# foxeng/libzseek

Measured on AMD Instinct MI355X. Metric: decompressed GB/s whole-node + achieved %HBM-read, LZ4 64KiB frames, higher is better.
Workload: dtype u8; 1 GPU; config2: LZ4 64KiB frames, 4 GiB synthetic per GPU, full-range decode, compressed image resident in HBM; frame_bytes=65536, frames_per_gpu=65536, decoded_bytes_total=4294967296, decoded_bytes_per_gpu=4294967296, compressed_bytes_per_gpu=2124820559, parallelism=one GPU

## Files before the change

### libzseek_amd/csrc/lz4_lean.hip

```cpp
#include <hip/hip_runtime.h>
#include <stdint.h>
#include <stdio.h>

#include "lz4_dev.h"
#include "zsk_internal.h"

namespace zsk {

namespace {

using namespace lz4d;

constexpr uint32_t kItemExt = 0x80000000u;
constexpr uint32_t kItemPos = 0x3FFFFFFFu;
constexpr uint32_t kLW = 4;
constexpr uint32_t kRing = 256;
constexpr uint32_t kMirror = 256, kSink = 272, kIBuf = 304;
constexpr uint32_t kStride = 560;
constexpr uint32_t kFlush = 8;
constexpr uint32_t kOff = 0x80000000u;

enum : uint32_t { P_TOKEN = 0, P_LEXT, P_OFF, P_MEXT, P_BHDR, P_END, P_DONE };

struct Fill {
    u32x4 a, b, c, d;
    uint32_t x;
    bool h2;
};

struct Lane {
    __amdgpu_buffer_rsrc_t cin, irs;
    uint32_t cx0;
    uint32_t clen, dlen;
    uint32_t ring;
    uint32_t fill, avail;
    uint32_t ph;
    int32_t st;
    uint32_t ip, op, fail_op;
    uint32_t csz_flag;
    uint64_t csize;
    uint32_t indep, bsid, max_block;
    uint32_t iend, oend, floor_, bop;
    uint32_t mlim;
    uint32_t tok, lsrc, nlit;
    uint32_t acc, moff;
    uint32_t stop;
    uint32_t ib, k, cap;
    uint32_t kf;
    uint32_t ia, ibw, ia2, ib2, nk;
    uint32_t cnt[22];
    uint32_t why;
};

constexpr int kLeanStats = 22;
__device__ unsigned long long g_lean_stats[kLeanStats];

__device__ __forceinline__ uint32_t lds_u32(uint32_t a)
{
    return *reinterpret_cast<const __attribute__((address_space(3))) uint32_t *>(
        (__attribute__((address_space(3))) void *)(uintptr_t)a);
}

__device__ __forceinline__ uint32_t lds_u8(uint32_t a)
{
    return *reinterpret_cast<const __attribute__((address_space(3))) uint8_t *>(
        (__attribute__((address_space(3))) void *)(uintptr_t)a);
}

template <typename T>
__device__ __forceinline__ __attribute__((address_space(3))) T *lp(uint32_t a)
{
    return (__attribute__((address_space(3))) T *)(uintptr_t)a;
}

__device__ __forceinline__ void lds_w128(uint32_t a, u32x4 v)
{
    *reinterpret_cast<__attribute__((address_space(3))) u32x4 *>(
        (__attribute__((address_space(3))) void *)(uintptr_t)a) = v;
}

__device__ __forceinline__ uint32_t raddr(const Lane &L, uint32_t x)
{
    return L.ring + (x & (kRing - 1));
}

__device__ __forceinline__ bool have(const Lane &L, uint32_t p, uint32_t n)
{
    return L.cx0 + p + n <= L.avail;
}

__device__ __forceinline__ uint32_t rb(const Lane &L, uint32_t p)
{
    return lds_u8(raddr(L, L.cx0 + p));
}

__device__ __forceinline__ uint32_t r4(const Lane &L, uint32_t p)
{
    const uint32_t x = L.cx0 + p;
    const uint32_t a = L.ring + (x & (kRing - 4));
    return __builtin_amdgcn_alignbyte(lds_u32(a + 4), lds_u32(a), x & 3);
}

__device__ __forceinline__ void ring_put(const Lane &L, uint32_t x, u32x4 a, u32x4 b, bool on)
{
    const uint32_t i = x & (kRing - 1);
    lds_w128(L.ring + (on ? i : kSink), a);
    lds_w128(L.ring + (on ? i + 16 : kSink + 16), b);
    lds_w128(L.ring + ((on && i == 0) ? kMirror : kSink), a);
}

__device__ __forceinline__ uint32_t rd32(const Lane &L, uint32_t p)
{
    return rb(L, p) | (rb(L, p + 1) << 8) | (rb(L, p + 2) << 16) | (rb(L, p + 3) << 24);
}

__device__ __forceinline__ u32x4 bload16(__amdgpu_buffer_rsrc_t r, uint32_t x)
{
    return __builtin_bit_cast(u32x4, __builtin_amdgcn_raw_buffer_load_b128(r, x, 0, 0));
}

__device__ __forceinline__ void finish(Lane &L, int32_t st)
{
    L.st = st;
    L.ph = P_DONE;
}

__device__ __forceinline__ void fail_block(Lane &L)
{
    const bool direct = (L.dlen - L.bop) >= L.max_block;
    const int32_t bits = (int32_t)((L.bsid - 4) << ST_BSID_SHIFT);
    finish(L, (direct ? (ST_GENERIC | ST_DIRECT_FLAG) : ST_DECOMPRESS_FAILED) | ST_BLOCK_FAIL_FLAG | bits);
}

__device__ __forceinline__ bool emit(Lane &L, uint32_t lsrc, uint32_t lit, uint32_t off, uint32_t ml)
{
    if (L.k + 2 > L.cap)
        return false;
    if (lit > 255 || ml > 258) {
        L.ia = lsrc | kItemExt;
        L.ibw = off;
        L.ia2 = lit;
        L.ib2 = ml;
        L.nk = 2;
    } else {
        L.ia = lsrc;
        L.ibw = off | (lit << 16) | ((ml ? ml - 3 : 0) << 24);
        L.ia2 = 0;
        L.ib2 = 0;
        L.nk = 1;
    }
    return true;
}

__device__ __forceinline__ int32_t hdr_status(Lane &L)
{
    const uint32_t clen = L.clen;
    if (clen < 7)
        return ST_HDR_INCOMPLETE;
    const uint32_t magic = rd32(L, 0);
    if ((magic & 0xFFFFFFF0u) == 0x184D2A50u)
        return ST_SHORT_FRAME;
    if (magic != kLz4Magic)
        return ST_FRAME_TYPE;
    const uint32_t flg = rb(L, 4), bd = rb(L, 5);
    if (flg & 0x14)
        return ST_NOT_RUN;
    const uint32_t dictid = flg & 1;
    if ((flg >> 1) & 1)
        return ST_RESERVED;
    if (((flg >> 6) & 3) != 1)
        return ST_VERSION;
    const uint32_t csz = (flg >> 3) & 1;
    const uint32_t hdr = 7 + (csz ? 8 : 0) + (dictid ? 4 : 0);
    if (clen < hdr)
        return ST_HDR_INCOMPLETE;
    const uint32_t bsid = (bd >> 4) & 7;
    if ((bd >> 7) & 1)
        return ST_RESERVED;
    if (bsid < 4)
        return ST_MAXBLOCK;
    if (bd & 15)
        return ST_RESERVED;
    const uint32_t n = hdr - 5;
    uint32_t acc = 0x165667B1u + n;
    uint32_t i = 0;
    for (; i + 4 <= n; i += 4) {
        acc += rd32(L, 4 + i) * 0xC2B2AE3Du;
        acc = ((acc << 17) | (acc >> 15)) * 0x27D4EB2Fu;
    }
    for (; i < n; i++) {
        acc += rb(L, 4 + i) * 0x165667B1u;
        acc = ((acc << 11) | (acc >> 21)) * 0x9E3779B1u;
    }
    acc ^= acc >> 15;
    acc *= 0x85EBCA77u;
    acc ^= acc >> 13;
    acc *= 0xC2B2AE3Du;
    acc ^= acc >> 16;
    if (((acc >> 8) & 0xFF) != rb(L, hdr - 1))
        return ST_HDR_CHECKSUM;
    L.indep = (flg >> 5) & 1;
    L.csz_flag = csz;
    L.bsid = bsid;
    if (csz)
        L.csize = (uint64_t)rd32(L, 6) | ((uint64_t)rd32(L, 10) << 32);
    L.max_block = 1u << (8 + 2 * bsid);
    L.ip = hdr;
    return -1;
}

template <bool FV = true>
__device__ __forceinline__ bool fast(Lane &L, uint32_t fe, uint32_t pc, u32x4 &fv)
{
    const uint32_t ip = L.ip, ph = L.ph;
    const bool po = ph == P_OFF;
    const uint32_t w = r4(L, ip);
    const uint32_t tok = w & 0xFF, e = (w >> 8) & 0xFF;
    const bool lext = (tok >> 4) == 15;
    const uint32_t lit = lext ? 15 + e : tok >> 4;
    const uint32_t p = ip + (lext ? 2 : 1);
    const uint32_t q = p + lit;
    if (FV)
        fv = *lp<u32x4>(fe + 16 * pc);
    const uint32_t o4q = r4(L, q);
    const uint32_t qq = po ? ip : q;
    const uint32_t o4 = po ? w : o4q;
    const uint32_t mtok = po ? L.tok : tok;
    const uint32_t off = o4 & 0xFFFF, e2 = (o4 >> 16) & 0xFF;
    const bool mext = (mtok & 15) == 15;
    const uint32_t ml = (mext ? 15 + e2 : mtok & 15) + kMinMatch;
    const uint32_t nip = qq + (mext ? 3 : 2);
    const uint32_t lt = po ? L.nlit : lit, ls = po ? L.lsrc : p;
    const uint32_t cop = po ? L.op : L.op + lit;
    const int32_t s_av = (int32_t)(L.avail - (L.cx0 + qq + 3));
    const int32_t s_in = (int32_t)(L.iend - qq - 8);
    const int32_t s_lx = (!po & lext & (e == 255)) ? -1 : 0, s_mx = (int32_t)(273 - ml);
    const int32_t s_mf = po ? 0 : (int32_t)(L.oend - kMfLimit - cop);
    const int32_t s_dl = po ? 0 : (int32_t)(L.dlen - cop);
    const int32_t s_off = min((int32_t)(off - 1), (int32_t)(cop - L.floor_ - off));
    const int32_t s_end = (int32_t)(L.mlim - cop - ml);
    const int32_t s_cap = (int32_t)(min(L.cap, L.kf + 32) - L.k - 2);
    const int32_t s_ph = ((ph == P_TOKEN) | po) ? 0 : -1;
    const int32_t s_t = min(min(s_in, s_dl), min(s_lx, s_mf));
    const int32_t slack = min(min(min(s_av, s_t), min(s_mx, s_off)), min(s_end, min(s_cap, s_ph)));
    const bool go = slack >= 0;
    const bool tok_av = (int32_t)(L.avail - (L.cx0 + ip + 2)) >= 0;
    const bool half = (ph == P_TOKEN) & tok_av & (s_t >= 0) & (s_av < 0);
    L.why = (s_av < 0) | (s_in < 0) << 1 | (s_lx < 0) << 2 | (s_mf < 0) << 3 | (s_mx < 0) << 4 |
            (s_off < 0) << 5 | (s_end < 0) << 6 | (s_cap < 0) << 7 | (!po & (ph != P_TOKEN)) << 8;
    const bool big = (lt > 255) | (ml > 258);
    L.ia = big ? ls | kItemExt : ls;
    L.ibw = big ? off : off | (lt << 16) | ((ml - 3) << 24);
    L.ia2 = lt;
    L.ib2 = ml;
    L.nk = go ? (big ? 2 : 1) : 0;
    L.ip = go ? nip : (half ? q : ip);
    L.op = go ? cop + ml : (half ? cop : L.op);
    L.lsrc = half ? p : L.lsrc;
    L.nlit = half ? lit : L.nlit;
    L.tok = half ? tok : L.tok;
    L.ph = go ? (uint32_t)P_TOKEN : (half ? (uint32_t)P_OFF : ph);
    const bool full = L.k + 2 > L.kf + 32;
    const bool wait = (!tok_av & (ip + 2 <= L.clen)) | full;
    const bool x_wait = (ph != P_END) & ((int32_t)(L.avail - (L.cx0 + ip + 4)) < 0) & (ip + 4 <= L.clen);
    return !go & !half & (ph != P_DONE) & (((ph != P_TOKEN) | po) ? !x_wait & !(po & full) : !wait);
}

__device__ __forceinline__ void lit_done(Lane &L, uint32_t p, uint32_t lit)
{
    if (L.op + lit > L.oend - kMfLimit || L.iend - p < lit + 2 + 1 + kLastLiterals) {
        if (L.iend - p != lit || L.op + lit > L.oend) {
            fail_block(L);
            return;
        }
        if (L.op + lit > L.dlen) {
            finish(L, ST_DST_OVERFLOW);
            return;
        }
        if (!emit(L, p, lit, 0, 0)) {
            finish(L, ST_NOT_RUN);
            return;
        }
        L.op += lit;
        L.ip = L.iend;
        L.ph = P_BHDR;
        return;
    }
    if (L.op + lit > L.dlen) {
        finish(L, ST_DST_OVERFLOW);
        return;
    }
    L.lsrc = p;
    L.nlit = lit;
    L.op += lit;
    L.ip = p + lit;
    L.ph = P_OFF;
}

__device__ __forceinline__ void match_done(Lane &L, uint32_t p, uint32_t off, uint32_t ml)
{
    ml += kMinMatch;
    if (off > L.op - L.floor_) {
        fail_block(L);
        return;
    }
    if (off == 0) {
        finish(L, ST_NOT_RUN);
        return;
    }
    if (L.op + ml > L.oend - kLastLiterals) {
        fail_block(L);
        return;
    }
    if (L.op + ml > L.dlen) {
        finish(L, ST_DST_OVERFLOW);
        return;
    }
    if (!emit(L, L.lsrc, L.nlit, off, ml)) {
        finish(L, ST_NOT_RUN);
        return;
    }
    L.op += ml;
    L.ip = p;
    L.ph = P_TOKEN;
}

__device__ __forceinline__ void slow(Lane &L)
{
    if (L.k + 2 > L.kf + 32)
        return;
    if (L.ph == P_TOKEN) {
        uint32_t p = L.ip;
        if (p >= L.iend) {
            fail_block(L);
            return;
        }
        if (!have(L, p, 1))
            return;
        const uint32_t tok = rb(L, p++);
        L.tok = tok;
        if ((tok >> 4) != 15) {
            lit_done(L, p, tok >> 4);
            return;
        }
        if (L.iend - p <= 15) {
            fail_block(L);
            return;
        }
        L.acc = 15;
        L.ip = p;
        L.ph = P_LEXT;
    }
    if (L.ph == P_LEXT) {
        uint32_t p = L.ip, lit = L.acc, e;
        do {
            if (p >= L.iend) {
                fail_block(L);
                return;
            }
            if (!have(L, p, 1)) {
                L.ip = p;
                L.acc = lit;
                return;
            }
            e = rb(L, p++);
            lit += e;
        } while (e == 255);
        lit_done(L, p, lit);
        return;
    }
    if (L.ph == P_OFF) {
        uint32_t p = L.ip;
        if (!have(L, p, 2))
            return;
        const uint32_t off = rb(L, p) | (rb(L, p + 1) << 8);
        p += 2;
        if ((L.tok & 15) != 15) {
            match_done(L, p, off, L.tok & 15);
            return;
        }
        L.moff = off;
        L.acc = 15;
        L.ip = p;
        L.ph = P_MEXT;
    }
    if (L.ph == P_MEXT) {
        uint32_t p = L.ip, ml = L.acc, e;
        do {
            if (p >= L.iend) {
                fail_block(L);
                return;
            }
            if (!have(L, p, 1)) {
                L.ip = p;
                L.acc = ml;
                return;
            }
            e = rb(L, p++);
            ml += e;
            if (p >= L.iend - (kLastLiterals - 1)) {
                fail_block(L);
                return;
            }
        } while (e == 255);
        match_done(L, p, L.moff, ml);
        return;
    }
    if (L.ph == P_BHDR) {
        if (L.ip == L.stop) {
            finish(L, ST_OK);
            return;
        }
        L.fail_op = L.op;
        if (L.clen - L.ip < 4) {
            finish(L, ST_TRUNCATED);
            return;
        }
        if (!have(L, L.ip, 4))
            return;
        const uint32_t bh = rd32(L, L.ip);
        L.ip += 4;
        if (bh == 0) {
            L.ph = P_END;
        } else {
            const uint32_t bsize = bh & 0x7FFFFFFFu;
            if (bsize > L.max_block) {
                finish(L, ST_MAXBLOCK);
                return;
            }
            if (L.clen - L.ip < bsize) {
                finish(L, ST_TRUNCATED);
                return;
            }
            L.bop = L.op;
            if (bh & 0x80000000u) {
                if (L.op + bsize > L.dlen) {
                    finish(L, ST_DST_OVERFLOW);
                    return;
                }
                if (!emit(L, L.ip, bsize, 0, 0)) {
                    finish(L, ST_NOT_RUN);
                    return;
                }
                L.op += bsize;
                L.ip += bsize;
                return;
            }
            if (bsize == 0) {
                fail_block(L);
                return;
            }
            L.iend = L.ip + bsize;
            L.oend = L.op + L.max_block;
            L.floor_ = L.indep ? L.op : 0;
            L.mlim = min(L.oend - kLastLiterals, L.dlen);
            L.ph = P_TOKEN;
            return;
        }
    }
    if (L.ph == P_END) {
        L.fail_op = L.op;
        if (L.csz_flag && L.csize != L.op)
            finish(L, ST_FRAME_SIZE);
        else
            finish(L, L.op != L.dlen ? ST_SHORT_FRAME : ST_OK);
    }
}

__device__ __forceinline__ uint32_t flush_hand(Lane &L, uint32_t tab)
{
    const bool ready = L.k - L.kf >= 16;
    const uint64_t rm = __ballot(ready);
    const uint32_t j = __builtin_amdgcn_mbcnt_hi((uint32_t)(rm >> 32), __builtin_amdgcn_mbcnt_lo((uint32_t)rm, 0u));
    const bool mine = ready && j < kFlush;
    const uint32_t line = L.ring + kIBuf + 128 * ((L.kf >> 4) & 1);
    *lp<uint64_t>(mine ? tab + 8 * j : tab + 8 * kFlush) = ((uint64_t)(8 * (L.ib + L.kf)) << 32) | line;
    L.kf = mine ? L.kf + 16 : L.kf;
    return min((uint32_t)__builtin_popcountll(rm), kFlush);
}

__device__ __forceinline__ void put_items(Lane &L)
{
    const uint32_t ibuf = L.ring + kIBuf;
    const uint32_t a0 = L.nk ? ibuf + 8 * (L.k & 31) : L.ring + kSink;
    const uint32_t a1 = L.nk == 2 ? ibuf + 8 * ((L.k + 1) & 31) : L.ring + kSink + 8;
    *lp<uint64_t>(a0) = ((uint64_t)L.ibw << 32) | L.ia;
    *lp<uint64_t>(a1) = ((uint64_t)L.ib2 << 32) | L.ia2;
    L.k += L.nk;
    L.nk = 0;
}

__device__ __forceinline__ void fill_retire(Lane &L, const Fill &S)
{
    const bool in = S.x == L.avail;
    ring_put(L, S.x, S.a, S.b, in);
    ring_put(L, S.x + 32, S.c, S.d, in && S.h2);
    L.avail = in ? L.avail + (S.h2 ? 64 : 32) : L.avail;
}

__device__ __forceinline__ void fill_issue(Lane &L, Fill &S, uint32_t need_x, bool live)
{
    const bool jump = need_x >= L.fill;
    L.fill = jump ? need_x & ~31u : L.fill;
    L.avail = jump ? L.fill : L.avail;
    const uint32_t lim = need_x + kRing - 16;
    const bool fl = live & (L.fill < L.cx0 + L.clen) & (L.fill + 32 <= lim);
    const bool f2 = fl & (L.fill + 32 < L.cx0 + L.clen) & (L.fill + 64 <= lim);
    const uint32_t fx = fl ? L.fill : kOff;
    S.x = fx;
    S.h2 = f2;
    S.a = bload16(L.cin, fx);
    S.b = bload16(L.cin, fl ? fx + 16 : kOff);
    S.c = bload16(L.cin, f2 ? fx + 32 : kOff);
    S.d = bload16(L.cin, f2 ? fx + 48 : kOff);
    L.fill = fl ? L.fill + (f2 ? 64 : 32) : L.fill;
}

template <int DIAG>
__device__ __forceinline__ void flush_store(const Lane &L, uint64_t fe, const u32x4 &fv, uint32_t g,
                                            uint32_t pc, uint32_t fcnt)
{
    const uint32_t at = (DIAG & 2) ? 16 * pc : (uint32_t)(fe >> 32) + 16 * pc;
    __builtin_amdgcn_raw_buffer_store_b128(__builtin_bit_cast(u32x4, fv), L.irs,
                                           g < fcnt && !(DIAG & 1) ? at : kOff, 0, 0);
}

template <bool SLOW, bool FILL, int DIAG>
__device__ __forceinline__ void sub(Lane &L, Fill &S, uint32_t lane, uint32_t tab, uint32_t &fcnt)
{
    if (FILL)
        fill_retire(L, S);
    const uint32_t g = lane >> 3, pc = lane & 7;
    const uint64_t fe = *lp<uint64_t>(tab + 8 * (g < fcnt ? g : kFlush));
    u32x4 fv;
    const bool need = fast(L, (uint32_t)fe, pc, fv);
    if (DIAG & 4) {
        L.cnt[0] += L.nk != 0;
        L.cnt[1] += need;
        L.cnt[2] += L.nk == 0 && !need && L.ph != P_DONE;
        L.cnt[3] += L.ph == P_DONE;
        if (need) {
            for (int b = 0; b < 9; b++)
                L.cnt[6 + b] += (L.why >> b) & 1;
            L.cnt[15 + min(L.ph, 6u)] += 1;
        }
    }
    flush_store<DIAG>(L, fe, fv, g, pc, fcnt);
    if (SLOW && __builtin_expect(__ballot(need) != 0, 0)) {
        if (DIAG & 4)
            L.cnt[4] += 1;
        if (need)
            slow(L);
    }
    put_items(L);
    if (!(DIAG & 32)) {
        u32x4 dv;
        (void)fast(L, L.ring + kSink, 0, dv);
        put_items(L);
    }
    wave_lds_sync();
    fcnt = flush_hand(L, tab);
    wave_lds_sync();
    if (!FILL)
        return;
    fill_issue(L, S, L.cx0 + L.ip, L.ph < P_END);
}

__device__ __forceinline__ bool lane_setup(Lane &L, const FrameDesc &d, bool act, uint64_t rb0, uint32_t cap,
                                           const uint8_t *comp, uint64_t *items, uint64_t capacity,
                                           uint64_t clo, uint64_t chi, uint64_t ilo, uint64_t ihi)
{
    const uintptr_t cbase = reinterpret_cast<uintptr_t>(comp + clo) & ~(uintptr_t)31;
    const uint64_t cspan = reinterpret_cast<uintptr_t>(comp + chi) - cbase;
    const uint64_t ispan = (ihi - ilo) * 8;
    const bool fits = cspan < 0x7FFFFF00ull && ispan < 0x7FFFFF00ull;
    L.cin = __builtin_amdgcn_make_buffer_rsrc((void *)cbase, 0, fits ? (int)(uint32_t)((cspan + 3) & ~3ull) : 0,
                                              kRsrcDw3);
    L.irs = __builtin_amdgcn_make_buffer_rsrc((void *)(items + ilo), 0, fits ? (int)(uint32_t)ispan : 0, kRsrcDw3);
    L.ib = (uint32_t)(rb0 - ilo);
    L.cx0 = (uint32_t)(reinterpret_cast<uintptr_t>(comp + d.c_off) - cbase);
    L.clen = d.c_size;
    L.dlen = d.d_size;
    L.fill = L.cx0 & ~31u;
    L.avail = L.fill;
    L.ph = P_BHDR;
    L.st = ST_NOT_RUN;
    L.ip = L.op = L.fail_op = 0;
    L.csz_flag = 0;
    L.csize = 0;
    L.indep = L.bsid = L.max_block = 0;
    L.iend = L.oend = L.floor_ = L.bop = L.mlim = 0;
    L.tok = L.lsrc = L.nlit = L.acc = L.moff = 0;
    L.k = L.kf = 0;
    L.stop = 0xFFFFFFFFu;
    L.cap = cap;
    L.ia = L.ibw = L.ia2 = L.ib2 = L.nk = 0;
    for (int i = 0; i < kLeanStats; i++)
        L.cnt[i] = 0;
    L.why = 0;
    return act && fits && d.c_size <= kItemPos && rb0 + cap <= capacity;
}

__device__ __forceinline__ void head_fill(Lane &L)
{
#pragma unroll
    for (int i = 0; i < 4; i++) {
        const uint32_t fx = L.fill;
        const u32x4 a = bload16(L.cin, fx), b = bload16(L.cin, fx + 16);
        ring_put(L, fx, a, b, true);
        L.fill += 32;
    }
    L.avail = L.fill;
}

template <int DIAG, int D, bool BLK>
__global__ __launch_bounds__(64 * kLW) __attribute__((amdgpu_waves_per_eu(1, 1))) void lz4_lean_kernel(
    const FrameDesc *__restrict__ desc, uint32_t n, const uint8_t *__restrict__ comp,
    const uint64_t *__restrict__ rec_base, uint64_t capacity, uint64_t *__restrict__ items,
    uint32_t *__restrict__ nitems, int32_t *__restrict__ status, uint32_t *__restrict__ fail_at,
    uint32_t max_csize, uint32_t min_csize, const BlockJob *__restrict__ jobs, BlockRes *__restrict__ jres,
    const uint32_t *__restrict__ njobs)
{
    __shared__ __attribute__((aligned(16))) uint8_t rings[kLW * 64 * kStride];
    __shared__ __attribute__((aligned(16))) uint64_t tabs[kLW * (kFlush + 1)];
    const uint32_t lane = threadIdx.x & 63;
    const uint32_t tab = (uint32_t)(uintptr_t)(tabs) + (threadIdx.x >> 6) * 8 * (kFlush + 1);
    const uint32_t f = blockIdx.x * (64 * kLW) + threadIdx.x;
    FrameDesc d = {0, 0, 0, 0};
    BlockJob J = {kNoJob, 0, 0, 0, 0, 0, 0, 0};
    bool act;
    if (BLK) {
        const uint32_t nj = uni(*njobs);
        if (nj >= min_csize && f < nj && f < n)
            J = jobs[f];
        act = J.f != kNoJob;
        if (act)
            d = desc[J.f];
    } else {
        if (f < n)
            d = desc[f];
        act = f < n && d.c_size < max_csize && d.c_size >= min_csize;
    }
    uint64_t rb0 = 0;
    uint32_t cap = 0;
    if (act) {
        rb0 = rec_base[BLK ? J.f : f] + J.slot_off * (uint32_t)BLK;
        cap = BLK ? J.slot_cap : slots_of(d.c_size);
    }
    const uint64_t clo = uni64(wave_min64(act ? d.c_off : ~0ull));
    const uint64_t chi = uni64(wave_max64(act ? d.c_off + d.c_size : 0ull));
    const uint64_t ilo = uni64(wave_min64(act ? rb0 : ~0ull));
    const uint64_t ihi = uni64(wave_max64(act ? rb0 + cap : 0ull));
    const uint64_t work = BLK ? (uint64_t)(J.stop - J.hpos) : (uint64_t)d.c_size;
    const uint32_t steps = (uint32_t)__builtin_amdgcn_readfirstlane(
        (int)(uint32_t)(wave_max64(act ? work : 0ull) * 2 + 64 * D + 1024));
    if (clo == ~0ull)
        return;
    Lane L;
    L.ring = (uint32_t)(uintptr_t)(rings) + threadIdx.x * kStride;
    if (!lane_setup(L, d, act, rb0, cap, comp, items, capacity, clo, chi, ilo, ihi)) {
        finish(L, ST_NOT_RUN);
    } else if (BLK) {
        L.ip = J.hpos;
        L.op = J.bop;
        L.stop = J.stop;
        L.bsid = J.info & 0xFF;
        L.indep = (J.info >> 8) & 1;
        L.max_block = 1u << (8 + 2 * L.bsid);
        L.fill = (L.cx0 + J.hpos) & ~31u;
        head_fill(L);
    } else {
        head_fill(L);
        const int32_t hs = hdr_status(L);
        if (hs >= 0)
            finish(L, hs);
    }
    Fill sl[D];
#pragma unroll
    for (int i = 0; i < D; i++) {
        sl[i].x = kOff;
        sl[i].h2 = false;
    }
    uint32_t rounds = 0, fcnt = 0;
    *lp<uint64_t>(tab + 8 * kFlush) = L.ring + kIBuf;
    wave_lds_sync();
    for (;;) {
        if (DIAG & 64) {
#pragma unroll
            for (int i = 0; i < D; i += 2) {
                sub<false, true, DIAG>(L, sl[i], lane, tab, fcnt);
                sub<true, true, DIAG>(L, sl[i + 1], lane, tab, fcnt);
            }
        } else {
#pragma unroll
            for (int i = 0; i < D; i++) {
                sub<false, true, DIAG>(L, sl[i], lane, tab, fcnt);
                sub<true, false, DIAG>(L, sl[i], lane, tab, fcnt);
            }
        }
        const bool busy = L.ph != P_DONE;
        if (!__any(busy))
            break;
        if (++rounds > steps) {
            if (busy)
                L.st = ST_NOT_RUN;
            break;
        }
    }
    {
        const uint32_t g = lane >> 3, pc = lane & 7;
        const uint64_t fe = *lp<uint64_t>(tab + 8 * (g < fcnt ? g : kFlush));
        const u32x4 fv = *lp<u32x4>((uint32_t)fe + 16 * pc);
        flush_store<DIAG>(L, fe, fv, g, pc, fcnt);
    }
    for (uint32_t x = L.kf; x < L.k; x += 2) {
        const uint32_t a = L.ring + kIBuf + 8 * (x & 31);
        const u32x4 v = (u32x4){lp<uint32_t>(a)[0], lp<uint32_t>(a)[1],
                                lp<uint32_t>(L.ring + kIBuf + 8 * ((x + 1) & 31))[0],
                                lp<uint32_t>(L.ring + kIBuf + 8 * ((x + 1) & 31))[1]};
        __builtin_amdgcn_raw_buffer_store_b128(__builtin_bit_cast(u32x4, v), L.irs, 8 * (L.ib + x), 0, 0);
    }
    if ((DIAG & 4) && act) {
        L.cnt[5] = L.k;
        for (int i = 0; i < kLeanStats; i++)
            atomicAdd(&g_lean_stats[i], (unsigned long long)L.cnt[i]);
    }
    if (!act)
        return;
    if (BLK) {
        jres[f] = BlockRes{L.k, L.op, L.st, 0};
        return;
    }
    status[f] = L.st;
    nitems[f] = L.k;
    if (fail_at)
        fail_at[f] = L.fail_op;
}

constexpr uint32_t kDone = 0x80000000u;
constexpr uint32_t kPairLds = kLW * 64 * kStride + kLW * 8 * (kFlush + 1) + kLW * 64 * 16;
static_assert(kPairLds <= 160 * 1024, "the pair parse's LDS exceeds a CU's 160 KB");

__device__ __forceinline__ void mail_put(uint32_t a, uint32_t lo, uint32_t hi)
{
    __hip_atomic_store(lp<uint64_t>(a), ((uint64_t)hi << 32) | lo, __ATOMIC_RELEASE, __HIP_MEMORY_SCOPE_WORKGROUP);
}

__device__ __forceinline__ uint64_t mail_get(uint32_t a)
{
    return __hip_atomic_load(lp<uint64_t>(a), __ATOMIC_ACQUIRE, __HIP_MEMORY_SCOPE_WORKGROUP);
}

template <bool SLOW, bool STATS>
__device__ __forceinline__ void parser_sub(Lane &L, uint32_t mp, uint32_t mm)
{
    const uint64_t m = mail_get(mm);
    L.avail = (uint32_t)m;
    L.kf = (uint32_t)(m >> 32);
    u32x4 dv;
    const bool live = L.ph != P_DONE;
    const bool need = fast<false>(L, 0, 0, dv);
    const bool e1 = L.nk != 0;
    if (STATS) {
        L.cnt[0] += live;
        L.cnt[1] += e1;
        L.cnt[3] += live && !e1 && !need && (L.why & 1);
        L.cnt[4] += live && !e1 && !need && (L.why & 128);
        L.cnt[5] += need;
    }
    if (SLOW && __builtin_expect(__ballot(need) != 0, 0)) {
        if (STATS)
            L.cnt[8] += 1;
        if (need)
            slow(L);
    }
    put_items(L);
    (void)fast<false>(L, 0, 0, dv);
    if (STATS) {
        L.cnt[2] += L.nk != 0;
        L.cnt[6] += e1 && L.nk == 0 && (L.why & 1);
        L.cnt[7] += e1 && L.nk == 0 && (L.why & 128);
    }
    put_items(L);
    mail_put(mp, L.cx0 + L.ip, L.k | (L.ph == P_DONE ? kDone : 0u));
}

template <bool FILL>
__device__ __forceinline__ void mover_sub(Lane &L, Fill &S, bool &done, uint32_t lane, uint32_t tab,
                                          uint32_t mp, uint32_t mm, uint32_t &fcnt)
{
    const uint64_t m = mail_get(mp);
    const uint32_t need_x = (uint32_t)m;
    L.k = (uint32_t)(m >> 32) & ~kDone;
    done = (m >> 63) != 0;
    if (FILL)
        fill_retire(L, S);
    const uint32_t g = lane >> 3, pc = lane & 7;
    const uint64_t fe = *lp<uint64_t>(tab + 8 * (g < fcnt ? g : kFlush));
    const u32x4 fv = *lp<u32x4>((uint32_t)fe + 16 * pc);
    mail_put(mm, L.avail, L.kf);
    flush_store<0>(L, fe, fv, g, pc, fcnt);
    wave_lds_sync();
    fcnt = flush_hand(L, tab);
    wave_lds_sync();
    if (FILL)
        fill_issue(L, S, need_x, !done);
}

template <bool EVERY, int D, bool STATS>
__global__ __launch_bounds__(128 * kLW) __attribute__((amdgpu_waves_per_eu(2, 2))) void lz4_lean_pair_kernel(
    const FrameDesc *__restrict__ desc, uint32_t n, const uint8_t *__restrict__ comp,
    const uint64_t *__restrict__ rec_base, uint64_t capacity, uint64_t *__restrict__ items,
    uint32_t *__restrict__ nitems, int32_t *__restrict__ status, uint32_t *__restrict__ fail_at,
    uint32_t max_csize, uint32_t min_csize)
{
    __shared__ __attribute__((aligned(16))) uint8_t rings[kLW * 64 * kStride];
    __shared__ __attribute__((aligned(16))) uint64_t tabs[kLW * (kFlush + 1)];
    __shared__ __attribute__((aligned(16))) uint64_t mail_p[kLW * 64], mail_m[kLW * 64];
    static_assert(sizeof(rings) + sizeof(tabs) + sizeof(mail_p) + sizeof(mail_m) == kPairLds, "LDS layout");
    constexpr int kPD = 2;
    const uint32_t t = threadIdx.x & (64 * kLW - 1), lane = threadIdx.x & 63;
    const bool mover = uni(threadIdx.x) >= 64 * kLW;
    const uint32_t tab = (uint32_t)(uintptr_t)(tabs) + (t >> 6) * 8 * (kFlush + 1);
    const uint32_t mp = (uint32_t)(uintptr_t)(mail_p) + 8 * t, mm = (uint32_t)(uintptr_t)(mail_m) + 8 * t;
    const uint32_t f = blockIdx.x * (64 * kLW) + t;
    FrameDesc d = {0, 0, 0, 0};
    if (f < n)
        d = desc[f];
    const bool act = f < n && d.c_size < max_csize && d.c_size >= min_csize;
    uint64_t rb0 = 0;
    uint32_t cap = 0;
    if (act) {
        rb0 = rec_base[f];
        cap = slots_of(d.c_size);
    }
    const uint64_t clo = uni64(wave_min64(act ? d.c_off : ~0ull));
    const uint64_t chi = uni64(wave_max64(act ? d.c_off + d.c_size : 0ull));
    const uint64_t ilo = uni64(wave_min64(act ? rb0 : ~0ull));
    const uint64_t ihi = uni64(wave_max64(act ? rb0 + cap : 0ull));
    const uint32_t steps = (uint32_t)__builtin_amdgcn_readfirstlane(
        (int)(uint32_t)(wave_max64(act ? (uint64_t)d.c_size : 0ull) * 2 + 64 * kPD + 1024));
    const bool some = clo != ~0ull;
    Lane L;
    L.ring = (uint32_t)(uintptr_t)(rings) + t * kStride;
    bool ok = false;
    if (some) {
        ok = lane_setup(L, d, act, rb0, cap, comp, items, capacity, clo, chi, ilo, ihi);
        if (!ok)
            finish(L, ST_NOT_RUN);
        if (mover) {
            if (ok)
                head_fill(L);
            mail_put(mm, L.avail, 0);
        } else {
            mail_put(mp, L.cx0, ok ? 0u : kDone);
        }
    }
    __syncthreads();
    if (some && mover) {
        Fill sl[D];
#pragma unroll
        for (int i = 0; i < D; i++) {
            sl[i].x = kOff;
            sl[i].h2 = false;
        }
        uint32_t rounds = 0, fcnt = 0;
        bool done = !ok;
        *lp<uint64_t>(tab + 8 * kFlush) = L.ring + kIBuf;
        wave_lds_sync();
        for (;;) {
#pragma unroll
            for (int i = 0; i < D; i++) {
                mover_sub<true>(L, sl[i], done, lane, tab, mp, mm, fcnt);
                if (!EVERY)
                    mover_sub<false>(L, sl[i], done, lane, tab, mp, mm, fcnt);
            }
            const bool more = !done || L.k - L.kf >= 16;
            if (!__any(more) || ++rounds > steps + D)
                break;
        }
        const uint32_t g = lane >> 3, pc = lane & 7;
        const uint64_t fe = *lp<uint64_t>(tab + 8 * (g < fcnt ? g : kFlush));
        const u32x4 fv = *lp<u32x4>((uint32_t)fe + 16 * pc);
        flush_store<0>(L, fe, fv, g, pc, fcnt);
        mail_put(mm, L.avail, L.kf);
    } else if (some) {
        L.avail = (uint32_t)mail_get(mm);
        if (ok) {
            const int32_t hs = hdr_status(L);
            if (hs >= 0)
                finish(L, hs);
        }
        uint32_t rounds = 0;
        for (;;) {
#pragma unroll
            for (int i = 0; i < kPD; i++) {
                parser_sub<false, STATS>(L, mp, mm);
                parser_sub<true, STATS>(L, mp, mm);
            }
            const bool busy = L.ph != P_DONE;
            if (!__any(busy))
                break;
            if (++rounds > steps) {
                if (busy)
                    L.st = ST_NOT_RUN;
                break;
            }
        }
        mail_put(mp, L.cx0 + L.ip, L.k | kDone);
    }
    __syncthreads();
    if (mover || !act)
        return;
    const uint32_t kf = (uint32_t)(mail_get(mm) >> 32);
    for (uint32_t x = kf; x < L.k; x += 2) {
        const uint32_t a = L.ring + kIBuf + 8 * (x & 31);
        const u32x4 v = (u32x4){lp<uint32_t>(a)[0], lp<uint32_t>(a)[1],
                                lp<uint32_t>(L.ring + kIBuf + 8 * ((x + 1) & 31))[0],
                                lp<uint32_t>(L.ring + kIBuf + 8 * ((x + 1) & 31))[1]};
        __builtin_amdgcn_raw_buffer_store_b128(__builtin_bit_cast(u32x4, v), L.irs, 8 * (L.ib + x), 0, 0);
    }
    status[f] = L.st;
    nitems[f] = L.k;
    if (fail_at)
        fail_at[f] = L.fail_op;
    if (STATS)
        for (int i = 0; i < 9; i++)
            atomicAdd(&g_lean_stats[i], (unsigned long long)L.cnt[i]);
}

}

int launch_lz4_lean(const FrameDesc *d_desc, uint32_t nframes, const uint8_t *d_comp,
                    const uint64_t *rec_base, uint64_t capacity, uint64_t *items, uint32_t *nitems,
                    int32_t *d_status, uint32_t *d_fail_at, hipStream_t stream, uint32_t max_csize,
                    int diag, uint32_t min_csize)
{
    if (nframes == 0)
        return 0;
    const uint32_t per = 64 * kLW;
    const dim3 grid((nframes + per - 1) / per);
#define ZSK_PAIR(E, P, S)                                                                                       \
    hipLaunchKernelGGL((lz4_lean_pair_kernel<E, P, S>), grid, dim3(2 * per), 0, stream, d_desc, nframes, d_comp, \
                       rec_base, capacity, items, nitems, d_status, d_fail_at, max_csize, min_csize)
#ifdef ZSK_TUNING
#define ZSK_LEAN(D, P)                                                                                         \
    hipLaunchKernelGGL((lz4_lean_kernel<D, P, false>), grid, dim3(per), 0, stream, d_desc, nframes, d_comp, rec_base, \
                       capacity, items, nitems, d_status, d_fail_at, max_csize, min_csize, nullptr, nullptr,       \
                       nullptr)
    if (!(diag & 128)) {
        if (diag & 4) {
            unsigned long long z[kLeanStats] = {0};
            (void)hipMemcpyToSymbolAsync(HIP_SYMBOL(g_lean_stats), z, sizeof(z), 0, hipMemcpyHostToDevice, stream);
            ZSK_PAIR(false, 2, true);
            (void)hipMemcpyFromSymbolAsync(z, HIP_SYMBOL(g_lean_stats), sizeof(z), 0, hipMemcpyDeviceToHost, stream);
            (void)hipStreamSynchronize(stream);
            const double fr = nframes;
            fprintf(stderr, "pair parse per frame: live sub-steps %.1f first emitted %.1f second emitted %.1f; first "
                            "waits: bytes %.1f flush %.1f exact-needed %.1f; second misses after a first: bytes %.1f "
                            "flush %.1f; exact-step runs %.1f\n", z[0] / fr, z[1] / fr, z[2] / fr, z[3] / fr, z[4] / fr,
                    z[5] / fr, z[6] / fr, z[7] / fr, z[8] / fr);
        } else if ((diag & 72) == 72)
            ZSK_PAIR(true, 4, false);
        else if (diag & 64)
            ZSK_PAIR(true, 2, false);
        else if (diag & 8)
            ZSK_PAIR(false, 4, false);
        else
            ZSK_PAIR(false, 2, false);
        return hipGetLastError() == hipSuccess ? 0 : -1;
    }
    if (diag & 4) {
        unsigned long long z[kLeanStats] = {0};
        (void)hipMemcpyToSymbolAsync(HIP_SYMBOL(g_lean_stats), z, sizeof(z), 0, hipMemcpyHostToDevice, stream);
        ZSK_LEAN(4, 2);
        (void)hipMemcpyFromSymbolAsync(z, HIP_SYMBOL(g_lean_stats), sizeof(z), 0, hipMemcpyDeviceToHost, stream);
        (void)hipStreamSynchronize(stream);
        const double fr = nframes;
        fprintf(stderr, "lean parse per frame: sub-steps fast %.1f exact-needed %.1f waiting %.1f done %.1f "
                        "exact-step runs %.1f items %.1f\n", z[0] / fr, z[1] / fr, z[2] / fr, z[3] / fr, z[4] / fr, z[5] / fr);
        fprintf(stderr, "  exact-needed rules per frame: av %.1f in %.1f lx %.1f mf %.1f mx %.1f off %.1f end %.1f cap %.1f "
                        "phase %.1f; by phase TOKEN %.1f LEXT %.1f OFF %.1f MEXT %.1f BHDR %.1f END %.1f DONE %.1f\n",
                z[6] / fr, z[7] / fr, z[8] / fr, z[9] / fr, z[10] / fr, z[11] / fr, z[12] / fr, z[13] / fr, z[14] / fr,
                z[15] / fr, z[16] / fr, z[17] / fr, z[18] / fr, z[19] / fr, z[20] / fr, z[21] / fr);
    } else if ((diag & 96) == 96)
        ZSK_LEAN(96, 4);
    else if (diag & 64)
        ZSK_LEAN(64, 4);
    else if (diag & 32)
        ZSK_LEAN(32, 2);
    else if (diag & 2)
        ZSK_LEAN(2, 2);
    else if (diag & 1)
        ZSK_LEAN(1, 2);
    else if (diag & 8)
        ZSK_LEAN(0, 4);
    else if (diag & 16)
        ZSK_LEAN(0, 1);
    else
        ZSK_LEAN(0, 2);
#undef ZSK_LEAN
#else
    (void)diag;
    ZSK_PAIR(false, 2, false);
#endif
#undef ZSK_PAIR
    return hipGetLastError() == hipSuccess ? 0 : -1;
}

int launch_lz4_lean_blocks(const FrameDesc *d_desc, const uint8_t *d_comp, const uint64_t *rec_base,
                           uint64_t capacity, uint64_t *items, const SplitScratch *s, uint32_t lanes,
                           uint32_t min_jobs, hipStream_t stream)
{
    if (lanes == 0)
        return 0;
    if (lanes > s->jobs_cap || !s->jobs || !s->jres || !s->njobs)
        return -1;
    const uint32_t per = 64 * kLW;
    hipLaunchKernelGGL((lz4_lean_kernel<0, 2, true>), dim3((lanes + per - 1) / per), dim3(per), 0, stream,
                       d_desc, lanes, d_comp, rec_base, capacity, items, nullptr, nullptr, nullptr, 0u,
                       min_jobs, s->jobs, s->jres, s->njobs);
    return hipGetLastError() == hipSuccess ? 0 : -1;
}

}
```

### libzseek_amd/csrc/tuning.hip

```cpp
#include <hip/hip_runtime.h>
#include <stdint.h>

#include <mutex>

#include "zsk_internal.h"

namespace zsk {

namespace {
std::mutex g_mu;
SplitScratch g_s;

int staged(int stages, int route, int tune, const FrameDesc *d_desc, uint32_t nframes,
           const uint8_t *d_comp, uint8_t *d_out, int32_t *d_status, hipStream_t stream)
{
    std::lock_guard<std::mutex> g(g_mu);
    if (split_scratch_reserve(&g_s, nframes, split_items_default(&g_s, nframes), stream) != 0)
        return -1;
    Lz4Request rq;
    rq.nframes = nframes;
    rq.route = route;
    rq.stages = stages;
    rq.tune = tune;
    return launch_lz4_split(rq, {d_desc, d_comp, d_out, d_status, nullptr}, stream, &g_s);
}
int overlapped(uint32_t K, const FrameDesc *d_desc, uint32_t nframes, const uint8_t *d_comp, uint8_t *d_out,
               int32_t *d_status, hipStream_t stream)
{
    std::lock_guard<std::mutex> g(g_mu);
    static hipStream_t ps = nullptr;
    static hipEvent_t ev[17];
    if (!ps) {
        if (hipStreamCreateWithFlags(&ps, hipStreamNonBlocking) != hipSuccess)
            return -1;
        for (auto &e : ev)
            if (hipEventCreateWithFlags(&e, hipEventDisableTiming) != hipSuccess)
                return -1;
    }
    if (K < 1 || K > 16)
        return -1;
    if (split_scratch_reserve(&g_s, nframes, split_items_default(&g_s, nframes), stream) != 0)
        return -1;
    Lz4Request plan_only;
    plan_only.nframes = nframes;
    plan_only.stages = 1;
    if (launch_lz4_split(plan_only, {d_desc, d_comp, d_out, d_status, nullptr}, stream, &g_s) != 0)
        return -1;
    if (hipEventRecord(ev[16], stream) != hipSuccess || hipStreamWaitEvent(ps, ev[16], 0) != hipSuccess)
        return -1;
    for (uint32_t c = 0; c < K; c++) {
        const uint32_t f0 = (uint32_t)((uint64_t)nframes * c / K), f1 = (uint32_t)((uint64_t)nframes * (c + 1) / K);
        if (launch_lz4_lean(d_desc + f0, f1 - f0, d_comp, g_s.rec_base + f0, (uint64_t)g_s.items_cap, g_s.items,
                            g_s.nitems + f0, d_status + f0, nullptr, ps, 0xFFFFFFFFu, 0, 0) != 0)
            return -1;
        if (hipEventRecord(ev[c], ps) != hipSuccess || hipStreamWaitEvent(stream, ev[c], 0) != hipSuccess)
            return -1;
        if (launch_seq_exec(d_desc + f0, f1 - f0, d_comp, d_out, g_s.rec_base + f0, g_s.items, g_s.nitems + f0,
                            d_status + f0, stream) != 0)
            return -1;
    }
    return 0;
}
}

int launch_lz4_frames_variant(int variant, const FrameDesc *d_desc, uint32_t nframes,
                              const uint8_t *d_comp, uint8_t *d_out, int32_t *d_status,
                              hipStream_t stream)
{
    if (nframes == 0)
        return 0;
    if (variant == 0)
        return launch_lz4_frames(d_desc, nframes, d_comp, d_out, d_status, nullptr, stream);
    if (variant >= 1 && variant <= 4)
        return launch_lz4_frames(d_desc, nframes, d_comp, d_out, d_status, nullptr, stream, variant);
    if (variant >= 10 && variant <= 14)
        return staged(3, variant - 10, 0, d_desc, nframes, d_comp, d_out, d_status, stream);
    if (variant == 20)
        return staged(4, ROUTE_AUTO, 0, d_desc, nframes, d_comp, d_out, d_status, stream);
    if ((variant & 0xF00) == 0x100)
        return staged(4, ROUTE_AUTO, (variant & 0x1FF) << 8, d_desc, nframes, d_comp, d_out, d_status,
                      stream);
    if ((variant & 0xF00) == 0x300)
        return staged(4, ROUTE_AUTO, (variant & 0x3FF) << 8, d_desc, nframes, d_comp, d_out, d_status, stream);
    if ((variant & 0xF00) == 0x200)
        return staged(3, ROUTE_LEAN, variant & 0xFF, d_desc, nframes, d_comp, d_out, d_status, stream);
    if (variant == 0x400)
        return staged(4, ROUTE_AUTO, 0x400 << 8, d_desc, nframes, d_comp, d_out, d_status, stream);
    if (variant == 0x401)
        return staged(15, ROUTE_AUTO, 0x400 << 8, d_desc, nframes, d_comp, d_out, d_status, stream);
    if (variant == 0x402)
        return staged(15, ROUTE_AUTO, 0, d_desc, nframes, d_comp, d_out, d_status, stream);
    if ((variant & 0xF00) == 0x700)
        return staged(4, ROUTE_AUTO, (variant & 0xFFF) << 8, d_desc, nframes, d_comp, d_out, d_status, stream);
    if ((variant & 0xF00) == 0x800)
        return staged(4, ROUTE_AUTO, (variant & 0xFFF) << 8, d_desc, nframes, d_comp, d_out, d_status, stream);
    if ((variant & 0xF00) == 0x600)
        return staged(4, ROUTE_AUTO, (variant & 0xFFF) << 8, d_desc, nframes, d_comp, d_out, d_status, stream);
    if ((variant & 0xF00) == 0x500)
        return overlapped((uint32_t)(variant & 0xFF), d_desc, nframes, d_comp, d_out, d_status, stream);
    return -1;
}

}
```

Baseline: 1274 GB/s.

## Template lean LZ4 ring on config; carry ring coordinates and widen pair-kernel fills

```diff
diff --git a/libzseek_amd/csrc/lean_ring.h b/libzseek_amd/csrc/lean_ring.h
--- /dev/null
+++ b/libzseek_amd/csrc/lean_ring.h
@@ -0,0 +1,37 @@
+#pragma once
+#include <stdint.h>
+
+namespace zsk {
+
+template <uint32_t R>
+struct LeanRing {
+    static_assert(R % 32 == 0 && R >= 256, "32-byte pieces; the head fill is 128 bytes");
+    static constexpr bool kPow2 = (R & (R - 1)) == 0;
+    static constexpr uint32_t kMaxAdv = 273 + 3, kSlack = 3;
+    static_assert(kPow2 || R + kSlack + kMaxAdv <= 2 * R, "one conditional subtract must cover the longest advance");
+    static constexpr uint32_t kMirror = R, kMirrorLen = 16;
+
+    static constexpr uint32_t of(uint32_t x) { return x % R; }
+
+    static constexpr uint32_t adv(uint32_t pos, uint32_t n)
+    {
+        const uint32_t x = pos + n;
+        if (kPow2)
+            return x & (R - 1);
+        return x - R < x ? x - R : x;
+    }
+
+    static constexpr uint32_t adv_lazy(uint32_t pos, uint32_t n) { return pos + n; }
+
+    static constexpr uint32_t read4_at(uint32_t pos) { return pos & ~3u; }
+    static constexpr uint32_t read4_pick(uint32_t lo, uint32_t hi, uint32_t pos)
+    {
+        const uint32_t s = 8 * (pos & 3);
+        return s ? (lo >> s) | (hi << (32 - s)) : lo;
+    }
+
+    static constexpr uint32_t piece_at(uint32_t pos0, uint32_t i) { return adv(pos0, 32 * i); }
+    static constexpr bool piece_mirrored(uint32_t pos) { return pos == 0; }
+};
+
+}
diff --git a/libzseek_amd/csrc/lz4_lean.hip b/libzseek_amd/csrc/lz4_lean.hip
--- a/libzseek_amd/csrc/lz4_lean.hip
+++ b/libzseek_amd/csrc/lz4_lean.hip
@@ -2,6 +2,7 @@
 #include <stdint.h>
 #include <stdio.h>
 
+#include "lean_ring.h"
 #include "lz4_dev.h"
 #include "zsk_internal.h"
 
@@ -14,18 +15,29 @@
 constexpr uint32_t kItemExt = 0x80000000u;
 constexpr uint32_t kItemPos = 0x3FFFFFFFu;
 constexpr uint32_t kLW = 4;
-constexpr uint32_t kRing = 256;
-constexpr uint32_t kMirror = 256, kSink = 272, kIBuf = 304;
-constexpr uint32_t kStride = 560;
+template <uint32_t R_, uint32_t SLOT_, bool WSINK_, bool CARRY_ = true>
+struct Cfg {
+    using Ring = LeanRing<R_>;
+    static constexpr uint32_t R = R_, kPieces = SLOT_ / 32;
+    static constexpr bool kWaveSink = WSINK_, kCarry = CARRY_;
+    static_assert(CARRY_ || Ring::kPow2, "masked coordinates need a power of two");
+    static constexpr uint32_t kMirror = Ring::kMirror, kSink = R_ + 16, kIBuf = kSink + (WSINK_ ? 0 : 32);
+    static constexpr uint32_t kStride = kIBuf + 256;
+    static_assert(SLOT_ % 32 == 0 && kPieces >= 1 && kPieces <= 4 && kStride % 16 == 0, "lane area");
+};
+using BlockCfg = Cfg<256, 64, false, false>;
+using PairCfg = Cfg<256, 96, false>;
 constexpr uint32_t kFlush = 8;
 constexpr uint32_t kOff = 0x80000000u;
 
 enum : uint32_t { P_TOKEN = 0, P_LEXT, P_OFF, P_MEXT, P_BHDR, P_END, P_DONE };
 
+template <uint32_t P>
 struct Fill {
-    u32x4 a, b, c, d;
+    u32x4 v[2 * P];
     uint32_t x;
-    bool h2;
+    uint32_t rx;
+    uint32_t n;
 };
 
 struct Lane {
@@ -33,7 +45,10 @@
     uint32_t cx0;
     uint32_t clen, dlen;
     uint32_t ring;
+    uint32_t sink;
     uint32_t fill, avail;
+    uint32_t rfill;
+    uint32_t rip;
     uint32_t ph;
     int32_t st;
     uint32_t ip, op, fail_op;
@@ -79,9 +94,10 @@
         (__attribute__((address_space(3))) void *)(uintptr_t)a) = v;
 }
 
+template <class C>
 __device__ __forceinline__ uint32_t raddr(const Lane &L, uint32_t x)
 {
-    return L.ring + (x & (kRing - 1));
+    return L.ring + C::Ring::of(x);
 }
 
 __device__ __forceinline__ bool have(const Lane &L, uint32_t p, uint32_t n)
@@ -89,29 +105,40 @@
     return L.cx0 + p + n <= L.avail;
 }
 
+template <class C>
 __device__ __forceinline__ uint32_t rb(const Lane &L, uint32_t p)
 {
-    return lds_u8(raddr(L, L.cx0 + p));
-}
-
-__device__ __forceinline__ uint32_t r4(const Lane &L, uint32_t p)
-{
-    const uint32_t x = L.cx0 + p;
-    const uint32_t a = L.ring + (x & (kRing - 4));
-    return __builtin_amdgcn_alignbyte(lds_u32(a + 4), lds_u32(a), x & 3);
-}
-
-__device__ __forceinline__ void ring_put(const Lane &L, uint32_t x, u32x4 a, u32x4 b, bool on)
-{
-    const uint32_t i = x & (kRing - 1);
-    lds_w128(L.ring + (on ? i : kSink), a);
-    lds_w128(L.ring + (on ? i + 16 : kSink + 16), b);
-    lds_w128(L.ring + ((on && i == 0) ? kMirror : kSink), a);
-}
-
+    return lds_u8(raddr<C>(L, L.cx0 + p));
+}
+
+template <class C>
+__device__ __forceinline__ uint32_t r4(const Lane &L, uint32_t pos)
+{
+    const uint32_t a = L.ring + (C::kCarry ? C::Ring::read4_at(pos) : pos & (C::R - 4));
+    return __builtin_amdgcn_alignbyte(lds_u32(a + 4), lds_u32(a), pos & 3);
+}
+
+template <class C>
+__device__ __forceinline__ void ring_put(const Lane &L, uint32_t pos, u32x4 a, u32x4 b, bool on)
+{
+    const uint32_t i = C::kCarry ? pos : pos & (C::R - 1);
+    const uint32_t at = L.ring + i;
+    lds_w128(on ? at : L.sink, a);
+    lds_w128(on ? at + 16 : L.sink + 16, b);
+    lds_w128((on && C::Ring::piece_mirrored(i)) ? L.ring + C::kMirror : L.sink, a);
+}
+
+template <class C>
 __device__ __forceinline__ uint32_t rd32(const Lane &L, uint32_t p)
 {
-    return rb(L, p) | (rb(L, p + 1) << 8) | (rb(L, p + 2) << 16) | (rb(L, p + 3) << 24);
+    return rb<C>(L, p) | (rb<C>(L, p + 1) << 8) | (rb<C>(L, p + 2) << 16) | (rb<C>(L, p + 3) << 24);
+}
+
+template <class C>
+__device__ __forceinline__ void rip_sync(Lane &L)
+{
+    if (C::kCarry)
+        L.rip = C::Ring::of(L.cx0 + L.ip);
 }
 
 __device__ __forceinline__ u32x4 bload16(__amdgpu_buffer_rsrc_t r, uint32_t x)
@@ -152,17 +179,18 @@
     return true;
 }
 
+template <class C>
 __device__ __forceinline__ int32_t hdr_status(Lane &L)
 {
     const uint32_t clen = L.clen;
     if (clen < 7)
         return ST_HDR_INCOMPLETE;
-    const uint32_t magic = rd32(L, 0);
+    const uint32_t magic = rd32<C>(L, 0);
     if ((magic & 0xFFFFFFF0u) == 0x184D2A50u)
         return ST_SHORT_FRAME;
     if (magic != kLz4Magic)
         return ST_FRAME_TYPE;
-    const uint32_t flg = rb(L, 4), bd = rb(L, 5);
+    const uint32_t flg = rb<C>(L, 4), bd = rb<C>(L, 5);
     if (flg & 0x14)
         return ST_NOT_RUN;
     const uint32_t dictid = flg & 1;
@@ -185,11 +213,11 @@
     uint32_t acc = 0x165667B1u + n;
     uint32_t i = 0;
     for (; i + 4 <= n; i += 4) {
-        acc += rd32(L, 4 + i) * 0xC2B2AE3Du;
+        acc += rd32<C>(L, 4 + i) * 0xC2B2AE3Du;
         acc = ((acc << 17) | (acc >> 15)) * 0x27D4EB2Fu;
     }
     for (; i < n; i++) {
-        acc += rb(L, 4 + i) * 0x165667B1u;
+        acc += rb<C>(L, 4 + i) * 0x165667B1u;
         acc = ((acc << 11) | (acc >> 21)) * 0x9E3779B1u;
     }
     acc ^= acc >> 15;
@@ -197,32 +225,35 @@
     acc ^= acc >> 13;
     acc *= 0xC2B2AE3Du;
     acc ^= acc >> 16;
-    if (((acc >> 8) & 0xFF) != rb(L, hdr - 1))
+    if (((acc >> 8) & 0xFF) != rb<C>(L, hdr - 1))
         return ST_HDR_CHECKSUM;
     L.indep = (flg >> 5) & 1;
     L.csz_flag = csz;
     L.bsid = bsid;
     if (csz)
-        L.csize = (uint64_t)rd32(L, 6) | ((uint64_t)rd32(L, 10) << 32);
+        L.csize = (uint64_t)rd32<C>(L, 6) | ((uint64_t)rd32<C>(L, 10) << 32);
     L.max_block = 1u << (8 + 2 * bsid);
     L.ip = hdr;
+    rip_sync<C>(L);
     return -1;
 }
 
-template <bool FV = true>
+template <class C, bool FV = true>
 __device__ __forceinline__ bool fast(Lane &L, uint32_t fe, uint32_t pc, u32x4 &fv)
 {
-    const uint32_t ip = L.ip, ph = L.ph;
+    using Ring = typename C::Ring;
+    const uint32_t ip = L.ip, ph = L.ph, rip = C::kCarry ? L.rip : L.cx0 + ip;
     const bool po = ph == P_OFF;
-    const uint32_t w = r4(L, ip);
+    const uint32_t w = r4<C>(L, rip);
     const uint32_t tok = w & 0xFF, e = (w >> 8) & 0xFF;
     const bool lext = (tok >> 4) == 15;
     const uint32_t lit = lext ? 15 + e : tok >> 4;
     const uint32_t p = ip + (lext ? 2 : 1);
     const uint32_t q = p + lit;
+    const uint32_t rq = C::kCarry ? Ring::adv(rip, (lext ? 2 : 1) + lit) : L.cx0 + q;
     if (FV)
         fv = *lp<u32x4>(fe + 16 * pc);
-    const uint32_t o4q = r4(L, q);
+    const uint32_t o4q = r4<C>(L, rq);
     const uint32_t qq = po ? ip : q;
     const uint32_t o4 = po ? w : o4q;
     const uint32_t mtok = po ? L.tok : tok;
@@ -230,6 +261,7 @@
     const bool mext = (mtok & 15) == 15;
     const uint32_t ml = (mext ? 15 + e2 : mtok & 15) + kMinMatch;
     const uint32_t nip = qq + (mext ? 3 : 2);
+    const uint32_t rnip = Ring::adv_lazy(po ? rip : rq, mext ? 3 : 2);
     const uint32_t lt = po ? L.nlit : lit, ls = po ? L.lsrc : p;
     const uint32_t cop = po ? L.op : L.op + lit;
     const int32_t s_av = (int32_t)(L.avail - (L.cx0 + qq + 3));
@@ -255,6 +287,8 @@
     L.ib2 = ml;
     L.nk = go ? (big ? 2 : 1) : 0;
     L.ip = go ? nip : (half ? q : ip);
+    if (C::kCarry)
+        L.rip = go ? rnip : (half ? rq : rip);
     L.op = go ? cop + ml : (half ? cop : L.op);
     L.lsrc = half ? p : L.lsrc;
     L.nlit = half ? lit : L.nlit;
@@ -325,6 +359,7 @@
     L.ph = P_TOKEN;
 }
 
+template <class C>
 __device__ __forceinline__ void slow(Lane &L)
 {
     if (L.k + 2 > L.kf + 32)
@@ -337,7 +372,7 @@
         }
         if (!have(L, p, 1))
             return;
-        const uint32_t tok = rb(L, p++);
+        const uint32_t tok = rb<C>(L, p++);
         L.tok = tok;
         if ((tok >> 4) != 15) {
             lit_done(L, p, tok >> 4);
@@ -363,7 +398,7 @@
                 L.acc = lit;
                 return;
             }
-            e = rb(L, p++);
+            e = rb<C>(L, p++);
             lit += e;
         } while (e == 255);
         lit_done(L, p, lit);
@@ -373,7 +408,7 @@
         uint32_t p = L.ip;
         if (!have(L, p, 2))
             return;
-        const uint32_t off = rb(L, p) | (rb(L, p + 1) << 8);
+        const uint32_t off = rb<C>(L, p) | (rb<C>(L, p + 1) << 8);
         p += 2;
         if ((L.tok & 15) != 15) {
             match_done(L, p, off, L.tok & 15);
@@ -396,7 +431,7 @@
                 L.acc = ml;
                 return;
             }
-            e = rb(L, p++);
+            e = rb<C>(L, p++);
             ml += e;
             if (p >= L.iend - (kLastLiterals - 1)) {
                 fail_block(L);
@@ -418,7 +453,7 @@
         }
         if (!have(L, L.ip, 4))
             return;
-        const uint32_t bh = rd32(L, L.ip);
+        const uint32_t bh = rd32<C>(L, L.ip);
         L.ip += 4;
         if (bh == 0) {
             L.ph = P_END;
@@ -467,53 +502,67 @@
     }
 }
 
+template <class C>
 __device__ __forceinline__ uint32_t flush_hand(Lane &L, uint32_t tab)
 {
     const bool ready = L.k - L.kf >= 16;
     const uint64_t rm = __ballot(ready);
     const uint32_t j = __builtin_amdgcn_mbcnt_hi((uint32_t)(rm >> 32), __builtin_amdgcn_mbcnt_lo((uint32_t)rm, 0u));
     const bool mine = ready && j < kFlush;
-    const uint32_t line = L.ring + kIBuf + 128 * ((L.kf >> 4) & 1);
+    const uint32_t line = L.ring + C::kIBuf + 128 * ((L.kf >> 4) & 1);
     *lp<uint64_t>(mine ? tab + 8 * j : tab + 8 * kFlush) = ((uint64_t)(8 * (L.ib + L.kf)) << 32) | line;
     L.kf = mine ? L.kf + 16 : L.kf;
     return min((uint32_t)__builtin_popcountll(rm), kFlush);
 }
 
+template <class C>
 __device__ __forceinline__ void put_items(Lane &L)
 {
-    const uint32_t ibuf = L.ring + kIBuf;
-    const uint32_t a0 = L.nk ? ibuf + 8 * (L.k & 31) : L.ring + kSink;
-    const uint32_t a1 = L.nk == 2 ? ibuf + 8 * ((L.k + 1) & 31) : L.ring + kSink + 8;
+    const uint32_t ibuf = L.ring + C::kIBuf;
+    const uint32_t a0 = L.nk ? ibuf + 8 * (L.k & 31) : L.sink;
+    const uint32_t a1 = L.nk == 2 ? ibuf + 8 * ((L.k + 1) & 31) : L.sink + 8;
     *lp<uint64_t>(a0) = ((uint64_t)L.ibw << 32) | L.ia;
     *lp<uint64_t>(a1) = ((uint64_t)L.ib2 << 32) | L.ia2;
     L.k += L.nk;
     L.nk = 0;
 }
 
-__device__ __forceinline__ void fill_retire(Lane &L, const Fill &S)
+template <class C>
+__device__ __forceinline__ void fill_retire(Lane &L, const Fill<C::kPieces> &S)
 {
     const bool in = S.x == L.avail;
-    ring_put(L, S.x, S.a, S.b, in);
-    ring_put(L, S.x + 32, S.c, S.d, in && S.h2);
-    L.avail = in ? L.avail + (S.h2 ? 64 : 32) : L.avail;
-}
-
-__device__ __forceinline__ void fill_issue(Lane &L, Fill &S, uint32_t need_x, bool live)
+#pragma unroll
+    for (uint32_t i = 0; i < C::kPieces; i++)
+        ring_put<C>(L, C::kCarry ? C::Ring::piece_at(S.rx, i) : S.x + 32 * i, S.v[2 * i], S.v[2 * i + 1],
+                    in && i < S.n);
+    L.avail = in ? L.avail + 32 * S.n : L.avail;
+}
+
+template <class C>
+__device__ __forceinline__ void fill_issue(Lane &L, Fill<C::kPieces> &S, uint32_t need_x, bool live)
 {
     const bool jump = need_x >= L.fill;
     L.fill = jump ? need_x & ~31u : L.fill;
+    if (C::kCarry)
+        L.rfill = jump ? C::Ring::of(L.fill) : L.rfill;
     L.avail = jump ? L.fill : L.avail;
-    const uint32_t lim = need_x + kRing - 16;
-    const bool fl = live & (L.fill < L.cx0 + L.clen) & (L.fill + 32 <= lim);
-    const bool f2 = fl & (L.fill + 32 < L.cx0 + L.clen) & (L.fill + 64 <= lim);
-    const uint32_t fx = fl ? L.fill : kOff;
-    S.x = fx;
-    S.h2 = f2;
-    S.a = bload16(L.cin, fx);
-    S.b = bload16(L.cin, fl ? fx + 16 : kOff);
-    S.c = bload16(L.cin, f2 ? fx + 32 : kOff);
-    S.d = bload16(L.cin, f2 ? fx + 48 : kOff);
-    L.fill = fl ? L.fill + (f2 ? 64 : 32) : L.fill;
+    const uint32_t lim = need_x + C::R - 16, end = L.cx0 + L.clen;
+    bool on = live;
+    uint32_t n = 0;
+#pragma unroll
+    for (uint32_t i = 0; i < C::kPieces; i++) {
+        on = on & (L.fill + 32 * i < end) & (L.fill + 32 * (i + 1) <= lim);
+        const uint32_t fx = on ? L.fill + 32 * i : kOff;
+        S.v[2 * i] = bload16(L.cin, fx);
+        S.v[2 * i + 1] = bload16(L.cin, on ? fx + 16 : kOff);
+        n += on;
+    }
+    S.x = n ? L.fill : kOff;
+    S.rx = C::kCarry ? L.rfill : 0;
+    S.n = n;
+    L.fill += 32 * n;
+    if (C::kCarry)
+        L.rfill = C::Ring::adv(L.rfill, 32 * n);
 }
 
 template <int DIAG>
@@ -525,15 +574,15 @@
                                            g < fcnt && !(DIAG & 1) ? at : kOff, 0, 0);
 }
 
-template <bool SLOW, bool FILL, int DIAG>
-__device__ __forceinline__ void sub(Lane &L, Fill &S, uint32_t lane, uint32_t tab, uint32_t &fcnt)
+template <class C, bool SLOW, bool FILL, int DIAG>
+__device__ __forceinline__ void sub(Lane &L, Fill<C::kPieces> &S, uint32_t lane, uint32_t tab, uint32_t &fcnt)
 {
     if (FILL)
-        fill_retire(L, S);
+        fill_retire<C>(L, S);
     const uint32_t g = lane >> 3, pc = lane & 7;
     const uint64_t fe = *lp<uint64_t>(tab + 8 * (g < fcnt ? g : kFlush));
     u32x4 fv;
-    const bool need = fast(L, (uint32_t)fe, pc, fv);
+    const bool need = fast<C>(L, (uint32_t)fe, pc, fv);
     if (DIAG & 4) {
         L.cnt[0] += L.nk != 0;
         L.cnt[1] += need;
@@ -549,21 +598,23 @@
     if (SLOW && __builtin_expect(__ballot(need) != 0, 0)) {
         if (DIAG & 4)
             L.cnt[4] += 1;
-        if (need)
-            slow(L);
-    }
-    put_items(L);
+        if (need) {
+            slow<C>(L);
+            rip_sync<C>(L);
+        }
+    }
+    put_items<C>(L);
     if (!(DIAG & 32)) {
         u32x4 dv;
-        (void)fast(L, L.ring + kSink, 0, dv);
-        put_items(L);
+        (void)fast<C>(L, L.sink, 0, dv);
+        put_items<C>(L);
     }
     wave_lds_sync();
-    fcnt = flush_hand(L, tab);
+    fcnt = flush_hand<C>(L, tab);
     wave_lds_sync();
     if (!FILL)
         return;
-    fill_issue(L, S, L.cx0 + L.ip, L.ph < P_END);
+    fill_issue<C>(L, S, L.cx0 + L.ip, L.ph < P_END);
 }
 
 __device__ __forceinline__ bool lane_setup(Lane &L, const FrameDesc &d, bool act, uint64_t rb0, uint32_t cap,
@@ -583,6 +634,7 @@
     L.dlen = d.d_size;
     L.fill = L.cx0 & ~31u;
     L.avail = L.fill;
+    L.rfill = L.rip = 0;
     L.ph = P_BHDR;
     L.st = ST_NOT_RUN;
     L.ip = L.op = L.fail_op = 0;
@@ -601,19 +653,23 @@
     return act && fits && d.c_size <= kItemPos && rb0 + cap <= capacity;
 }
 
+template <class C>
 __device__ __forceinline__ void head_fill(Lane &L)
 {
+    L.rfill = C::kCarry ? C::Ring::of(L.fill) : 0;
 #pragma unroll
     for (int i = 0; i < 4; i++) {
         const uint32_t fx = L.fill;
         const u32x4 a = bload16(L.cin, fx), b = bload16(L.cin, fx + 16);
-        ring_put(L, fx, a, b, true);
+        ring_put<C>(L, C::kCarry ? L.rfill : fx, a, b, true);
         L.fill += 32;
+        if (C::kCarry)
+            L.rfill = C::Ring::adv(L.rfill, 32);
     }
     L.avail = L.fill;
 }
 
-template <int DIAG, int D, bool BLK>
+template <class C, int DIAG, int D, bool BLK>
 __global__ __launch_bounds__(64 * kLW) __attribute__((amdgpu_waves_per_eu(1, 1))) void lz4_lean_kernel(
     const FrameDesc *__restrict__ desc, uint32_t n, const uint8_t *__restrict__ comp,
     const uint64_t *__restrict__ rec_base, uint64_t capacity, uint64_t *__restrict__ items,
@@ -621,7 +677,7 @@
     uint32_t max_csize, uint32_t min_csize, const BlockJob *__restrict__ jobs, BlockRes *__restrict__ jres,
     const uint32_t *__restrict__ njobs)
 {
-    __shared__ __attribute__((aligned(16))) uint8_t rings[kLW * 64 * kStride];
+    __shared__ __attribute__((aligned(16))) uint8_t rings[kLW * 64 * C::kStride];
     __shared__ __attribute__((aligned(16))) uint64_t tabs[kLW * (kFlush + 1)];
     const uint32_t lane = threadIdx.x & 63;
     const uint32_t tab = (uint32_t)(uintptr_t)(tabs) + (threadIdx.x >> 6) * 8 * (kFlush + 1);
@@ -657,7 +713,9 @@
     if (clo == ~0ull)
         return;
     Lane L;
-    L.ring = (uint32_t)(uintptr_t)(rings) + threadIdx.x * kStride;
+    static_assert(!C::kWaveSink, "the single-wave kernel keeps a sink per lane");
+    L.ring = (uint32_t)(uintptr_t)(rings) + threadIdx.x * C::kStride;
+    L.sink = L.ring + C::kSink;
     if (!lane_setup(L, d, act, rb0, cap, comp, items, capacity, clo, chi, ilo, ihi)) {
         finish(L, ST_NOT_RUN);
     } else if (BLK) {
@@ -668,34 +726,35 @@
         L.indep = (J.info >> 8) & 1;
         L.max_block = 1u << (8 + 2 * L.bsid);
         L.fill = (L.cx0 + J.hpos) & ~31u;
-        head_fill(L);
+        head_fill<C>(L);
+        rip_sync<C>(L);
     } else {
-        head_fill(L);
-        const int32_t hs = hdr_status(L);
+        head_fill<C>(L);
+        const int32_t hs = hdr_status<C>(L);
         if (hs >= 0)
             finish(L, hs);
     }
-    Fill sl[D];
+    Fill<C::kPieces> sl[D];
 #pragma unroll
     for (int i = 0; i < D; i++) {
         sl[i].x = kOff;
-        sl[i].h2 = false;
+        sl[i].rx = sl[i].n = 0;
     }
     uint32_t rounds = 0, fcnt = 0;
-    *lp<uint64_t>(tab + 8 * kFlush) = L.ring + kIBuf;
+    *lp<uint64_t>(tab + 8 * kFlush) = L.ring + C::kIBuf;
     wave_lds_sync();
     for (;;) {
         if (DIAG & 64) {
 #pragma unroll
             for (int i = 0; i < D; i += 2) {
-                sub<false, true, DIAG>(L, sl[i], lane, tab, fcnt);
-                sub<true, true, DIAG>(L, sl[i + 1], lane, tab, fcnt);
+                sub<C, false, true, DIAG>(L, sl[i], lane, tab, fcnt);
+                sub<C, true, true, DIAG>(L, sl[i + 1], lane, tab, fcnt);
             }
         } else {
 #pragma unroll
             for (int i = 0; i < D; i++) {
-                sub<false, true, DIAG>(L, sl[i], lane, tab, fcnt);
-                sub<true, false, DIAG>(L, sl[i], lane, tab, fcnt);
+                sub<C, false, true, DIAG>(L, sl[i], lane, tab, fcnt);
+                sub<C, true, false, DIAG>(L, sl[i], lane, tab, fcnt);
             }
         }
         const bool busy = L.ph != P_DONE;
@@ -714,10 +773,10 @@
         flush_store<DIAG>(L, fe, fv, g, pc, fcnt);
     }
     for (uint32_t x = L.kf; x < L.k; x += 2) {
-        const uint32_t a = L.ring + kIBuf + 8 * (x & 31);
+        const uint32_t a = L.ring + C::kIBuf + 8 * (x & 31);
         const u32x4 v = (u32x4){lp<uint32_t>(a)[0], lp<uint32_t>(a)[1],
-                                lp<uint32_t>(L.ring + kIBuf + 8 * ((x + 1) & 31))[0],
-                                lp<uint32_t>(L.ring + kIBuf + 8 * ((x + 1) & 31))[1]};
+                                lp<uint32_t>(L.ring + C::kIBuf + 8 * ((x + 1) & 31))[0],
+                                lp<uint32_t>(L.ring + C::kIBuf + 8 * ((x + 1) & 31))[1]};
         __builtin_amdgcn_raw_buffer_store_b128(__builtin_bit_cast(u32x4, v), L.irs, 8 * (L.ib + x), 0, 0);
     }
     if ((DIAG & 4) && act) {
@@ -738,8 +797,12 @@
 }
 
 constexpr uint32_t kDone = 0x80000000u;
-constexpr uint32_t kPairLds = kLW * 64 * kStride + kLW * 8 * (kFlush + 1) + kLW * 64 * 16;
-static_assert(kPairLds <= 160 * 1024, "the pair parse's LDS exceeds a CU's 160 KB");
+template <class C>
+constexpr uint32_t pair_lds()
+{
+    return kLW * 64 * C::kStride + kLW * 8 * (kFlush + 1) + kLW * 64 * 16 + 2 * kLW * 32;
+}
+static_assert(pair_lds<PairCfg>() <= 160 * 1024, "the pair parse's LDS exceeds a CU's 160 KB");
 
 __device__ __forceinline__ void mail_put(uint32_t a, uint32_t lo, uint32_t hi)
 {
@@ -751,7 +814,7 @@
     return __hip_atomic_load(lp<uint64_t>(a), __ATOMIC_ACQUIRE, __HIP_MEMORY_SCOPE_WORKGROUP);
 }
 
-template <bool SLOW, bool STATS>
+template <class C, bool SLOW, bool STATS>
 __device__ __forceinline__ void parser_sub(Lane &L, uint32_t mp, uint32_t mm)
 {
     const uint64_t m = mail_get(mm);
@@ -759,7 +822,7 @@
     L.kf = (uint32_t)(m >> 32);
     u32x4 dv;
     const bool live = L.ph != P_DONE;
-    const bool need = fast<false>(L, 0, 0, dv);
+    const bool need = fast<C, false>(L, 0, 0, dv);
     const bool e1 = L.nk != 0;
     if (STATS) {
         L.cnt[0] += live;
@@ -771,22 +834,24 @@
     if (SLOW && __builtin_expect(__ballot(need) != 0, 0)) {
         if (STATS)
             L.cnt[8] += 1;
-        if (need)
-            slow(L);
-    }
-    put_items(L);
-    (void)fast<false>(L, 0, 0, dv);
+        if (need) {
+            slow<C>(L);
+            rip_sync<C>(L);
+        }
+    }
+    put_items<C>(L);
+    (void)fast<C, false>(L, 0, 0, dv);
     if (STATS) {
         L.cnt[2] += L.nk != 0;
         L.cnt[6] += e1 && L.nk == 0 && (L.why & 1);
         L.cnt[7] += e1 && L.nk == 0 && (L.why & 128);
     }
-    put_items(L);
+    put_items<C>(L);
     mail_put(mp, L.cx0 + L.ip, L.k | (L.ph == P_DONE ? kDone : 0u));
 }
 
-template <bool FILL>
-__device__ __forceinline__ void mover_sub(Lane &L, Fill &S, bool &done, uint32_t lane, uint32_t tab,
+template <class C, bool FILL>
+__device__ __forceinline__ void mover_sub(Lane &L, Fill<C::kPieces> &S, bool &done, uint32_t lane, uint32_t tab,
                                           uint32_t mp, uint32_t mm, uint32_t &fcnt)
 {
     const uint64_t m = mail_get(mp);
@@ -794,30 +859,33 @@
     L.k = (uint32_t)(m >> 32) & ~kDone;
     done = (m >> 63) != 0;
     if (FILL)
-        fill_retire(L, S);
+        fill_retire<C>(L, S);
     const uint32_t g = lane >> 3, pc = lane & 7;
     const uint64_t fe = *lp<uint64_t>(tab + 8 * (g < fcnt ? g : kFlush));
     const u32x4 fv = *lp<u32x4>((uint32_t)fe + 16 * pc);
     mail_put(mm, L.avail, L.kf);
     flush_store<0>(L, fe, fv, g, pc, fcnt);
     wave_lds_sync();
-    fcnt = flush_hand(L, tab);
+    fcnt = flush_hand<C>(L, tab);
     wave_lds_sync();
     if (FILL)
-        fill_issue(L, S, need_x, !done);
-}
-
-template <bool EVERY, int D, bool STATS>
+        fill_issue<C>(L, S, need_x, !done);
+}
+
+template <class C, bool EVERY, int D, bool STATS>
 __global__ __launch_bounds__(128 * kLW) __attribute__((amdgpu_waves_per_eu(2, 2))) void lz4_lean_pair_kernel(
     const FrameDesc *__restrict__ desc, uint32_t n, const uint8_t *__restrict__ comp,
     const uint64_t *__restrict__ rec_base, uint64_t capacity, uint64_t *__restrict__ items,
     uint32_t *__restrict__ nitems, int32_t *__restrict__ status, uint32_t *__restrict__ fail_at,
     uint32_t max_csize, uint32_t min_csize)
 {
-    __shared__ __attribute__((aligned(16))) uint8_t rings[kLW * 64 * kStride];
+    __shared__ __attribute__((aligned(16))) uint8_t rings[kLW * 64 * C::kStride];
     __shared__ __attribute__((aligned(16))) uint64_t tabs[kLW * (kFlush + 1)];
     __shared__ __attribute__((aligned(16))) uint64_t mail_p[kLW * 64], mail_m[kLW * 64];
-    static_assert(sizeof(rings) + sizeof(tabs) + sizeof(mail_p) + sizeof(mail_m) == kPairLds, "LDS layout");
+    __shared__ __attribute__((aligned(16))) uint8_t sinks[2 * kLW * 32];
+    static_assert(sizeof(rings) + sizeof(tabs) + sizeof(mail_p) + sizeof(mail_m) + sizeof(sinks) == pair_lds<C>(),
+                  "LDS layout");
+    static_assert(pair_lds<C>() <= 160 * 1024, "the pair parse's LDS exceeds a CU's 160 KB");
     constexpr int kPD = 2;
     const uint32_t t = threadIdx.x & (64 * kLW - 1), lane = threadIdx.x & 63;
     const bool mover = uni(threadIdx.x) >= 64 * kLW;
@@ -842,7 +910,8 @@
         (int)(uint32_t)(wave_max64(act ? (uint64_t)d.c_size : 0ull) * 2 + 64 * kPD + 1024));
     const bool some = clo != ~0ull;
     Lane L;
-    L.ring = (uint32_t)(uintptr_t)(rings) + t * kStride;
+    L.ring = (uint32_t)(uintptr_t)(rings) + t * C::kStride;
+    L.sink = C::kWaveSink ? (uint32_t)(uintptr_t)(sinks) + (threadIdx.x >> 6) * 32 : L.ring + C::kSink;
     bool ok = false;
     if (some) {
         ok = lane_setup(L, d, act, rb0, cap, comp, items, capacity, clo, chi, ilo, ihi);
@@ -850,7 +919,7 @@
             finish(L, ST_NOT_RUN);
         if (mover) {
             if (ok)
-                head_fill(L);
+                head_fill<C>(L);
             mail_put(mm, L.avail, 0);
         } else {
             mail_put(mp, L.cx0, ok ? 0u : kDone);
@@ -858,22 +927,22 @@
     }
     __syncthreads();
     if (some && mover) {
-        Fill sl[D];
+        Fill<C::kPieces> sl[D];
 #pragma unroll
         for (int i = 0; i < D; i++) {
             sl[i].x = kOff;
-            sl[i].h2 = false;
+            sl[i].rx = sl[i].n = 0;
         }
         uint32_t rounds = 0, fcnt = 0;
         bool done = !ok;
-        *lp<uint64_t>(tab + 8 * kFlush) = L.ring + kIBuf;
+        *lp<uint64_t>(tab + 8 * kFlush) = L.ring + C::kIBuf;
         wave_lds_sync();
         for (;;) {
 #pragma unroll
             for (int i = 0; i < D; i++) {
-                mover_sub<true>(L, sl[i], done, lane, tab, mp, mm, fcnt);
+                mover_sub<C, true>(L, sl[i], done, lane, tab, mp, mm, fcnt);
                 if (!EVERY)
-                    mover_sub<false>(L, sl[i], done, lane, tab, mp, mm, fcnt);
+                    mover_sub<C, false>(L, sl[i], done, lane, tab, mp, mm, fcnt);
             }
             const bool more = !done || L.k - L.kf >= 16;
             if (!__any(more) || ++rounds > steps + D)
@@ -887,7 +956,7 @@
     } else if (some) {
         L.avail = (uint32_t)mail_get(mm);
         if (ok) {
-            const int32_t hs = hdr_status(L);
+            const int32_t hs = hdr_status<C>(L);
             if (hs >= 0)
                 finish(L, hs);
         }
@@ -895,8 +964,8 @@
         for (;;) {
 #pragma unroll
             for (int i = 0; i < kPD; i++) {
-                parser_sub<false, STATS>(L, mp, mm);
-                parser_sub<true, STATS>(L, mp, mm);
+                parser_sub<C, false, STATS>(L, mp, mm);
+                parser_sub<C, true, STATS>(L, mp, mm);
             }
             const bool busy = L.ph != P_DONE;
             if (!__any(busy))
@@ -914,10 +983,10 @@
         return;
     const uint32_t kf = (uint32_t)(mail_get(mm) >> 32);
     for (uint32_t x = kf; x < L.k; x += 2) {
-        const uint32_t a = L.ring + kIBuf + 8 * (x & 31);
+        const uint32_t a = L.ring + C::kIBuf + 8 * (x & 31);
         const u32x4 v = (u32x4){lp<uint32_t>(a)[0], lp<uint32_t>(a)[1],
-                                lp<uint32_t>(L.ring + kIBuf + 8 * ((x + 1) & 31))[0],
-                                lp<uint32_t>(L.ring + kIBuf + 8 * ((x + 1) & 31))[1]};
+                                lp<uint32_t>(L.ring + C::kIBuf + 8 * ((x + 1) & 31))[0],
+                                lp<uint32_t>(L.ring + C::kIBuf + 8 * ((x + 1) & 31))[1]};
         __builtin_amdgcn_raw_buffer_store_b128(__builtin_bit_cast(u32x4, v), L.irs, 8 * (L.ib + x), 0, 0);
     }
     status[f] = L.st;
@@ -940,19 +1009,43 @@
         return 0;
     const uint32_t per = 64 * kLW;
     const dim3 grid((nframes + per - 1) / per);
-#define ZSK_PAIR(E, P, S)                                                                                       \
-    hipLaunchKernelGGL((lz4_lean_pair_kernel<E, P, S>), grid, dim3(2 * per), 0, stream, d_desc, nframes, d_comp, \
+#define ZSK_PAIR(C, E, P, S)                                                                                       \
+    hipLaunchKernelGGL((lz4_lean_pair_kernel<C, E, P, S>), grid, dim3(2 * per), 0, stream, d_desc, nframes, d_comp, \
                        rec_base, capacity, items, nitems, d_status, d_fail_at, max_csize, min_csize)
 #ifdef ZSK_TUNING
 #define ZSK_LEAN(D, P)                                                                                         \
-    hipLaunchKernelGGL((lz4_lean_kernel<D, P, false>), grid, dim3(per), 0, stream, d_desc, nframes, d_comp, rec_base, \
-                       capacity, items, nitems, d_status, d_fail_at, max_csize, min_csize, nullptr, nullptr,       \
-                       nullptr)
+    hipLaunchKernelGGL((lz4_lean_kernel<BlockCfg, D, P, false>), grid, dim3(per), 0, stream, d_desc, nframes, d_comp, \
+                       rec_base, capacity, items, nitems, d_status, d_fail_at, max_csize, min_csize, nullptr,      \
+                       nullptr, nullptr)
     if (!(diag & 128)) {
+        using R256 = Cfg<256, 64, false>;
+        using R256w = Cfg<256, 96, false>;
+        using R288 = Cfg<288, 64, false>;
+        using R288w = Cfg<288, 96, false>;
+        using R320 = Cfg<320, 64, true>;
+        using R320w = Cfg<320, 96, true>;
+        using R256x = Cfg<256, 128, false>;
+        using R320x = Cfg<320, 128, true>;
+        const int ring = diag & 0x33;
         if (diag & 4) {
             unsigned long long z[kLeanStats] = {0};
             (void)hipMemcpyToSymbolAsync(HIP_SYMBOL(g_lean_stats), z, sizeof(z), 0, hipMemcpyHostToDevice, stream);
-            ZSK_PAIR(false, 2, true);
+            if (ring == 0x01)
+                ZSK_PAIR(R256w, false, 2, true);
+            else if (ring == 0x10)
+                ZSK_PAIR(R288, false, 2, true);
+            else if (ring == 0x11)
+                ZSK_PAIR(R288w, false, 2, true);
+            else if (ring == 0x20)
+                ZSK_PAIR(R320, false, 2, true);
+            else if (ring == 0x21)
+                ZSK_PAIR(R320w, false, 2, true);
+            else if (ring == 0x02)
+                ZSK_PAIR(R256x, false, 2, true);
+            else if (ring == 0x22)
+                ZSK_PAIR(R320x, false, 2, true);
+            else
+                ZSK_PAIR(R256, false, 2, true);
             (void)hipMemcpyFromSymbolAsync(z, HIP_SYMBOL(g_lean_stats), sizeof(z), 0, hipMemcpyDeviceToHost, stream);
             (void)hipStreamSynchronize(stream);
             const double fr = nframes;
@@ -960,14 +1053,28 @@
                             "waits: bytes %.1f flush %.1f exact-needed %.1f; second misses after a first: bytes %.1f "
                             "flush %.1f; exact-step runs %.1f\n", z[0] / fr, z[1] / fr, z[2] / fr, z[3] / fr, z[4] / fr,
                     z[5] / fr, z[6] / fr, z[7] / fr, z[8] / fr);
-        } else if ((diag & 72) == 72)
-            ZSK_PAIR(true, 4, false);
+        } else if (ring == 0x01)
+            ZSK_PAIR(R256w, false, 2, false);
+        else if (ring == 0x10)
+            ZSK_PAIR(R288, false, 2, false);
+        else if (ring == 0x11)
+            ZSK_PAIR(R288w, false, 2, false);
+        else if (ring == 0x20)
+            ZSK_PAIR(R320, false, 2, false);
+        else if (ring == 0x21)
+            ZSK_PAIR(R320w, false, 2, false);
+        else if (ring == 0x02)
+            ZSK_PAIR(R256x, false, 2, false);
+        else if (ring == 0x22)
+            ZSK_PAIR(R320x, false, 2, false);
+        else if ((diag & 72) == 72)
+            ZSK_PAIR(R256, true, 4, false);
         else if (diag & 64)
-            ZSK_PAIR(true, 2, false);
+            ZSK_PAIR(R256, true, 2, false);
         else if (diag & 8)
-            ZSK_PAIR(false, 4, false);
+            ZSK_PAIR(R256, false, 4, false);
         else
-            ZSK_PAIR(false, 2, false);
+            ZSK_PAIR(R256, false, 2, false);
         return hipGetLastError() == hipSuccess ? 0 : -1;
     }
     if (diag & 4) {
@@ -1002,7 +1109,7 @@
 #undef ZSK_LEAN
 #else
     (void)diag;
-    ZSK_PAIR(false, 2, false);
+    ZSK_PAIR(PairCfg, false, 2, false);
 #endif
 #undef ZSK_PAIR
     return hipGetLastError() == hipSuccess ? 0 : -1;
@@ -1017,7 +1124,7 @@
     if (lanes > s->jobs_cap || !s->jobs || !s->jres || !s->njobs)
         return -1;
     const uint32_t per = 64 * kLW;
-    hipLaunchKernelGGL((lz4_lean_kernel<0, 2, true>), dim3((lanes + per - 1) / per), dim3(per), 0, stream,
+    hipLaunchKernelGGL((lz4_lean_kernel<BlockCfg, 0, 2, true>), dim3((lanes + per - 1) / per), dim3(per), 0, stream,
                        d_desc, lanes, d_comp, rec_base, capacity, items, nullptr, nullptr, nullptr, 0u,
                        min_jobs, s->jobs, s->jres, s->njobs);
     return hipGetLastError() == hipSuccess ? 0 : -1;
diff --git a/libzseek_amd/csrc/tuning.hip b/libzseek_amd/csrc/tuning.hip
--- a/libzseek_amd/csrc/tuning.hip
+++ b/libzseek_amd/csrc/tuning.hip
@@ -84,6 +84,8 @@
         return staged(4, ROUTE_AUTO, (variant & 0x3FF) << 8, d_desc, nframes, d_comp, d_out, d_status, stream);
     if ((variant & 0xF00) == 0x200)
         return staged(3, ROUTE_LEAN, variant & 0xFF, d_desc, nframes, d_comp, d_out, d_status, stream);
+    if ((variant & 0xF00) == 0x900)
+        return staged(15, ROUTE_LEAN, variant & 0xFF, d_desc, nframes, d_comp, d_out, d_status, stream);
     if (variant == 0x400)
         return staged(4, ROUTE_AUTO, 0x400 << 8, d_desc, nframes, d_comp, d_out, d_status, stream);
     if (variant == 0x401)
```

New measurement: 1298 GB/s, median of 6. 1.9% higher.
